# yamoling/lle

Measured on AMD Instinct MI355X. Metric: env-steps/s (agents x envs x steps/s), level-6 batch 65536, higher is better.
Workload: dtype u8

## Files before the change

lle_amd/csrc/obs_stream.hpp:

```cpp
#pragma once
#include <hip/hip_runtime.h>
#include <stdint.h>

#include <type_traits>

#include "tables.h"

namespace lle {

__device__ __forceinline__ void wave_sync() {
    __builtin_amdgcn_fence(__ATOMIC_RELEASE, "wavefront");
    __builtin_amdgcn_wave_barrier();
    __builtin_amdgcn_fence(__ATOMIC_ACQUIRE, "wavefront");
}

__device__ __forceinline__ uint32_t xcd_block(uint32_t b, uint32_t n_blocks) {
    const uint32_t x = b & 7u, q = n_blocks >> 3, r = n_blocks & 7u;
    return x * q + (x < r ? x : r) + (b >> 3);
}
__device__ __forceinline__ uint32_t xcd_block_dir(uint32_t b, uint32_t n_blocks, uint32_t flags) {
    const uint32_t blk = xcd_block(b, n_blocks);
    return (flags & LAUNCH_REVERSE) ? n_blocks - 1u - blk : blk;
}

__device__ __forceinline__ uint32_t row_rotation(uint32_t wave_id, uint32_t rows_per_wave, int64_t n_here, uint32_t flags) {
    const uint32_t r = wave_id & (rows_per_wave - 1u);
    return ((flags & LAUNCH_ROTATE_ROWS) && (int64_t)r < n_here && n_here == (int64_t)rows_per_wave) ? r : 0u;
}
__device__ __forceinline__ uint32_t rotated(uint32_t k, uint32_t rot, uint32_t n) {
    const uint32_t kk = k + rot;
    return kk >= n ? kk - n : kk;
}

typedef uint32_t u32x4 __attribute__((ext_vector_type(4)));
#define LLE_COPY_ROWS(SRC)                                                                                              \
    for (uint32_t r0 = wave_in_wg; r0 < rows; r0 += 8 * waves_per_wg) {                                                \
        const uint32_t r1 = r0 + waves_per_wg, r2 = r1 + waves_per_wg, r3 = r2 + waves_per_wg, r4 = r3 + waves_per_wg, \
                       r5 = r4 + waves_per_wg, r6 = r5 + waves_per_wg, r7 = r6 + waves_per_wg;                          \
        const u32x4 z = {0, 0, 0, 0};                                                                                   \
        u32x4 v0 = SRC(r0), v1 = z, v2 = z, v3 = z, v4 = z, v5 = z, v6 = z, v7 = z;                                      \
        if (r1 < rows) v1 = SRC(r1);                                                                                    \
        if (r2 < rows) v2 = SRC(r2);                                                                                    \
        if (r3 < rows) v3 = SRC(r3);                                                                                    \
        if (r4 < rows) {                                                                                                \
            v4 = SRC(r4);                                                                                               \
            if (r5 < rows) v5 = SRC(r5);                                                                                \
            if (r6 < rows) v6 = SRC(r6);                                                                                \
            if (r7 < rows) v7 = SRC(r7);                                                                                \
        }                                                                                                               \
        __builtin_amdgcn_sched_barrier(0);                        \
        dst[r0 * 64] = v0;                                                                                              \
        if (r1 < rows) dst[r1 * 64] = v1;                                                                               \
        if (r2 < rows) dst[r2 * 64] = v2;                                                                               \
        if (r3 < rows) dst[r3 * 64] = v3;                                                                               \
        if (r4 < rows) {                                                                                                \
            dst[r4 * 64] = v4;                                                                                          \
            if (r5 < rows) dst[r5 * 64] = v5;                                                                           \
            if (r6 < rows) dst[r6 * 64] = v6;                                                                           \
            if (r7 < rows) dst[r7 * 64] = v7;                                                                           \
        }                                                                                                               \
    }
__device__ __forceinline__ void copy_tables_to_lds(const uint8_t* __restrict__ tables, uint8_t* lds, uint32_t tab_bytes,
                                                   uint32_t lane, uint32_t wave_in_wg, uint32_t waves_per_wg) {
    const u32x4* __restrict__ src = reinterpret_cast<const u32x4*>(tables) + lane;
    u32x4* dst = reinterpret_cast<u32x4*>(lds) + lane;
    const uint32_t rows = tab_bytes / 1024;
#define LLE_SRC1(r) src[(r) * 64]
    LLE_COPY_ROWS(LLE_SRC1)
#undef LLE_SRC1
}

__device__ __forceinline__ void copy_tables2_to_lds(const uint8_t* __restrict__ t1, uint32_t bytes1, const uint8_t* __restrict__ t2, uint32_t bytes2,
                                                    uint8_t* lds, uint32_t lane, uint32_t wave_in_wg, uint32_t waves_per_wg) {
    const u32x4* __restrict__ s1 = reinterpret_cast<const u32x4*>(t1) + lane;
    const u32x4* __restrict__ s2 = reinterpret_cast<const u32x4*>(t2) + lane;
    u32x4* dst = reinterpret_cast<u32x4*>(lds) + lane;
    const uint32_t rows1 = bytes1 / 1024, rows = rows1 + bytes2 / 1024;
#define LLE_SRC2(r) (*((r) < rows1 ? s1 + (r) * 64 : s2 + ((r) - rows1) * 64))
    LLE_COPY_ROWS(LLE_SRC2)
#undef LLE_SRC2
}
#undef LLE_COPY_ROWS

__device__ __forceinline__ void expand_packed_tables(const uint8_t* __restrict__ pk, uint8_t* lds, uint32_t HW, uint32_t n_lay, uint32_t lds_meta, uint32_t lds_dyn,
                                                     uint32_t tail_bytes, uint32_t tid, uint32_t T) {
    const uint64_t* __restrict__ m4 = reinterpret_cast<const uint64_t*>(pk);
    const uint16_t* __restrict__ idx = reinterpret_cast<const uint16_t*>(pk + packed_meta_bytes(HW));
    const uint64_t* __restrict__ lay = reinterpret_cast<const uint64_t*>(pk + packed_meta_bytes(HW) + packed_idx_bytes(n_lay));
    const uint4* __restrict__ tail = reinterpret_cast<const uint4*>(pk + packed_meta_bytes(HW) + packed_idx_bytes(n_lay) + ((n_lay * 8u + 15u) & ~15u));
    const uint32_t n4 = (HW + 3u) / 4u, nt = tail_bytes / 16u;
    const uint64_t w0 = tid < n4 ? m4[tid] : 0ull;
    const uint32_t i0 = tid < n_lay ? (uint32_t)idx[tid] : 0u;
    const uint64_t l0 = tid < n_lay ? lay[tid] : 0ull;
    uint4 t0 = {0u, 0u, 0u, 0u};
    if (tid < nt) t0 = tail[tid];
    auto widen = [](uint64_t w) { return uint4{(uint32_t)w & 0xFFFFu, (uint32_t)(w >> 16) & 0xFFFFu, (uint32_t)(w >> 32) & 0xFFFFu, (uint32_t)(w >> 48)}; };
    uint4* z = reinterpret_cast<uint4*>(lds);
    for (uint32_t i = tid; i < lds_meta / 16u; i += T) z[i] = uint4{0u, 0u, 0u, 0u};
    uint4* md = reinterpret_cast<uint4*>(lds + lds_meta);
    if (tid < n4) md[tid] = widen(w0);
    for (uint32_t i = tid + T; i < n4; i += T) md[i] = widen(m4[i]);
    uint4* td = reinterpret_cast<uint4*>(lds + lds_dyn);
    if (tid < nt) td[tid] = t0;
    for (uint32_t i = tid + T; i < nt; i += T) td[i] = tail[i];
    asm volatile("s_waitcnt lgkmcnt(0)\n\ts_barrier" ::: "memory");
    uint64_t* ld = reinterpret_cast<uint64_t*>(lds);
    if (tid < n_lay) ld[i0] = l0;
    for (uint32_t i = tid + T; i < n_lay; i += T) ld[idx[i]] = lay[i];
}

__device__ __forceinline__ uint32_t mad24(uint32_t a, uint32_t b, uint32_t c) {
    uint32_t r;
    asm("v_mad_u32_u24 %0, %1, %2, %3" : "=v"(r) : "v"(a), "v"(b), "v"(c));
    return r;
}

template <typename T>
__device__ __forceinline__ void small_store(T* p, T v) {
#ifdef LLE_SMALL_WT
    if constexpr (sizeof(T) == 1) {
        asm volatile("global_store_byte %0, %1, off sc1" ::"v"(p), "v"((uint32_t)(uint8_t)v) : "memory");
    } else if constexpr (sizeof(T) == 2) {
        asm volatile("global_store_short %0, %1, off sc1" ::"v"(p), "v"((uint32_t)(uint16_t)v) : "memory");
    } else if constexpr (sizeof(T) == 4) {
        uint32_t w;
        __builtin_memcpy(&w, &v, 4);
        asm volatile("global_store_dword %0, %1, off sc1" ::"v"(p), "v"(w) : "memory");
    } else {
        static_assert(sizeof(T) == 8, "small_store: 1, 2, 4 or 8 bytes");
        uint64_t w;
        __builtin_memcpy(&w, &v, 8);
        asm volatile("global_store_dwordx2 %0, %1, off sc1" ::"v"(p), "v"(w) : "memory");
    }
#else
    *p = v;
#endif
}

template <bool WT>
__device__ __forceinline__ void stream_store(uint4* p, const uint4& v) {
    if constexpr (WT) {
        const u32x4 w = {v.x, v.y, v.z, v.w};
        asm volatile("global_store_dwordx4 %0, %1, off sc1\n\ts_nop 1" ::"v"(p), "v"(w));
    } else {
        *p = v;
    }
}

template <bool WT>
__device__ __forceinline__ void stream_row(uint4* __restrict__ dst, const uint4* srcv, uint32_t first, uint32_t n_chunks, uint32_t lane) {
    uint32_t c = first + lane;
    for (; c + 192u < n_chunks; c += 256u) {
        const uint4 q0 = srcv[c], q1 = srcv[c + 64u], q2 = srcv[c + 128u], q3 = srcv[c + 192u];
        stream_store<WT>(dst + c, q0);
        stream_store<WT>(dst + c + 64u, q1);
        stream_store<WT>(dst + c + 128u, q2);
        stream_store<WT>(dst + c + 192u, q3);
    }
    for (; c < n_chunks; c += 64u) stream_store<WT>(dst + c, srcv[c]);
}

template <bool WT>
__device__ __forceinline__ void stream_whole_row(uint4* __restrict__ dst, const uint4* srcv, uint32_t n_chunks, uint32_t lane) {
    const uint32_t c0 = lane, c1 = lane + 64u;
    const uint4 v0 = srcv[c0 < n_chunks ? c0 : 0u], v1 = srcv[c1 < n_chunks ? c1 : 0u];
    if (c0 < n_chunks) stream_store<WT>(dst + c0, v0);
    if (c1 < n_chunks) stream_store<WT>(dst + c1, v1);
    if (n_chunks > 128u) stream_row<WT>(dst, srcv, 128u, n_chunks, lane);
}

template <bool WT>
__device__ __forceinline__ void stream_row_tail(uint4* __restrict__ dst, const uint4* srcv, uint32_t n_chunks, uint32_t head_lo, uint32_t head_n,
                                                uint32_t lane, uint32_t head2_lo = 0, uint32_t head2_n = 0) {
    const uint32_t n_tail = n_chunks - head_n - head2_n;
    auto chunk_of = [&](uint32_t i) {
        uint32_t c = i + (i >= head_lo ? head_n : 0u);
        if (head2_n) c += c >= head2_lo ? head2_n : 0u;
        return c;
    };
    const uint32_t i0 = lane, i1 = lane + 64u;
    const uint32_t c0 = chunk_of(i0), c1 = chunk_of(i1);
    const uint4 v0 = srcv[i0 < n_tail ? c0 : 0u], v1 = srcv[i1 < n_tail ? c1 : 0u];
    if (i0 < n_tail) stream_store<WT>(dst + c0, v0);
    if (i1 < n_tail) stream_store<WT>(dst + c1, v1);
    for (uint32_t i = lane + 128u; i < n_tail; i += 64u) {
        const uint32_t c = chunk_of(i);
        stream_store<WT>(dst + c, srcv[c]);
    }
}

template <bool WT>
__device__ __forceinline__ void stream_row_dyn(uint4* __restrict__ dst, const uint4* srcv, const uint16_t* tab, uint32_t n_dyn, uint32_t c0, uint32_t c1,
                                               uint32_t lane) {
    const uint4 v0 = srcv[c0 != 0xFFFFu ? c0 : 0u], v1 = srcv[c1 != 0xFFFFu ? c1 : 0u];
    if (c0 != 0xFFFFu) stream_store<WT>(dst + c0, v0);
    if (c1 != 0xFFFFu) stream_store<WT>(dst + c1, v1);
    for (uint32_t i = lane + 128u; i < n_dyn; i += 64u) {
        const uint32_t c = tab[i];
        stream_store<WT>(dst + c, srcv[c]);
    }
}

__device__ __forceinline__ uint4 widen_chunk16(const int8_t* tmpl, uint32_t q, uint32_t one, uint32_t sel_lo, uint32_t sel_hi) {
    const uint2 w = reinterpret_cast<const uint2*>(tmpl)[q];
    uint32_t o[4];
#pragma unroll
    for (int k = 0; k < 4; k++) {
        const uint32_t src = k < 2 ? w.x : w.y;
        const uint32_t x = __builtin_amdgcn_perm(src, src, (k & 1) ? sel_hi : sel_lo);
        o[k] = __umul24(x & 0x00010001u, one) | ((x & 0x00800080u) << 8);
    }
    return make_uint4(o[0], o[1], o[2], o[3]);
}
__device__ __forceinline__ uint4 widen_chunk32(const int8_t* tmpl, uint32_t q) {
    const uint32_t w = reinterpret_cast<const uint32_t*>(tmpl)[q];
    uint32_t o[4];
#pragma unroll
    for (int k = 0; k < 4; k++) {
        const uint32_t b = (w >> (8 * k)) & 0xFFu;
        o[k] = ((b & 1u) ? 0x3F800000u : 0u) | ((b & 0x80u) << 24);
    }
    return make_uint4(o[0], o[1], o[2], o[3]);
}
struct WideConsts { uint32_t one, sel_lo, sel_hi, sh, lane; };
__device__ __forceinline__ WideConsts wide_consts(uint32_t et, uint32_t lane) {
    uint32_t z = 0;
    asm volatile("" : "+s"(z));
    asm volatile("" : "+v"(lane));
    WideConsts c;
    c.one = (et == OBS_F16 ? 0x3C00u : 0x3F80u) | z;
    c.sel_lo = 0x0c010c00u | z;
    c.sel_hi = 0x0c030c02u | z;
    c.sh = obs_elem_shift(et) + z;
    c.lane = lane;
    return c;
}
template <bool WT>
__device__ __forceinline__ void stream_wide(uint4* __restrict__ dst, const int8_t* tmpl, uint32_t n_chunks, uint32_t et, uint32_t lane_in) {
    const WideConsts c = wide_consts(et, lane_in);
    const uint32_t n_out = n_chunks << c.sh;
    if (c.sh == 2u) {
#pragma clang loop unroll(disable)
        for (uint32_t q = c.lane; q < n_out; q += 64u) stream_store<WT>(dst + q, widen_chunk32(tmpl, q));
    } else {
#pragma clang loop unroll(disable)
        for (uint32_t q = c.lane; q < n_out; q += 64u) stream_store<WT>(dst + q, widen_chunk16(tmpl, q, c.one, c.sel_lo, c.sel_hi));
    }
}
template <bool WT>
__device__ __forceinline__ void stream_wide_dyn(uint4* __restrict__ dst, const int8_t* tmpl, const uint16_t* tab, uint32_t t_lo, uint32_t t_hi, uint32_t c_base,
                                                uint32_t et, uint32_t lane_in) {
    const WideConsts c = wide_consts(et, lane_in);
#pragma clang loop unroll(disable)
    for (uint32_t i = (t_lo << c.sh) + c.lane; i < (t_hi << c.sh); i += 64u) {
        const uint32_t q = (((uint32_t)tab[i >> c.sh] - c_base) << c.sh) + (i & ((1u << c.sh) - 1u));
        stream_store<WT>(dst + q, c.sh == 2u ? widen_chunk32(tmpl, q) : widen_chunk16(tmpl, q, c.one, c.sel_lo, c.sel_hi));
    }
}

template <bool WT>
__device__ __forceinline__ void store_heads(int8_t* __restrict__ obs, uint64_t obs_stride, int64_t env0, int64_t n_here, uint32_t head_lo,
                                            uint32_t head_n, const uint4& v, uint32_t lane, uint32_t rot = 0, uint32_t head2_lo = 0, uint32_t head2_n = 0) {
    const uint32_t chunk = lane < head_n ? head_lo + lane : head2_lo + (lane - head_n);
    if (lane < head_n + head2_n)
        for (uint32_t k = 0; k < (uint32_t)n_here; k++)
            stream_store<WT>(reinterpret_cast<uint4*>(obs + (uint64_t)(env0 + rotated(k, rot, (uint32_t)n_here)) * obs_stride) + chunk, v);
}

template <bool CAN_WIDE, typename F>
__device__ __forceinline__ void dispatch_stream(uint32_t lflags, F&& f) {
    const bool wt = (lflags & LAUNCH_WRITE_THROUGH) != 0;
    if constexpr (CAN_WIDE) {
        if (lflags & LAUNCH_OBS_ELEM_MASK) {
            if (wt) f(std::true_type{}, std::true_type{});
            else f(std::false_type{}, std::true_type{});
            return;
        }
    }
    if (wt) f(std::true_type{}, std::false_type{});
    else f(std::false_type{}, std::false_type{});
}

template <bool WT, bool HEAD = false, bool INCR = false, bool WIDE = false>
__device__ __forceinline__ void write_observations(int A, int L, uint32_t D, uint32_t n_chunks, uint64_t obs_stride,
                                                   const uint64_t* dyn, int8_t* tmpl, const uint32_t* scratch,
                                                   uint32_t scr_stride, int8_t* __restrict__ obs, int64_t env0,
                                                   int64_t n_here, uint32_t lane, uint32_t head_lo = 0, uint32_t head_n = 0, uint32_t rot = 0,
                                                   const uint16_t* dyn_chunks = nullptr, uint32_t n_dyn_chunks = 0, uint32_t et = OBS_I8) {
    static_assert(!(WIDE && HEAD), "the kernels with row heads carry no widening code: the launcher never sends them a widened launch");
    uint32_t dc0 = 0xFFFFu, dc1 = 0xFFFFu;
    if constexpr (INCR) {
        dc0 = lane < n_dyn_chunks ? (uint32_t)dyn_chunks[lane] : 0xFFFFu;
        dc1 = lane + 64u < n_dyn_chunks ? (uint32_t)dyn_chunks[lane + 64u] : 0xFFFFu;
    }
    const bool has_d0 = lane < D;
    const uint64_t e0 = has_d0 ? dyn[lane] : 0ull;
    const uint32_t d0_idx = dyn_index(e0);
    const int32_t d0_base = dyn_base(e0);
    const uint32_t d0_refs = dyn_refs(e0), d0_gem = dyn_gem(e0);
    const uint32_t d0_r0 = dyn_ref0(e0), d0_r1 = dyn_ref1(e0);
    const uint32_t d0_w0 = d0_refs >= 1 ? 1u + ref_word(d0_r0) : 0u, d0_s0 = d0_refs >= 1 ? ref_bit(d0_r0) : 0u;
    const uint32_t d0_w1 = d0_refs >= 2 ? 1u + ref_word(d0_r1) : 0u, d0_s1 = d0_refs >= 2 ? ref_bit(d0_r1) : 0u;
    const uint32_t d0_wg = d0_gem != NO_GEM ? (uint32_t)L + 1u : 0u, d0_sg = d0_gem != NO_GEM ? gem_bit(d0_gem) : 0u;
    const bool is_agent_lane = (int)lane < A;
    const uint4* srcv = reinterpret_cast<const uint4*>(tmpl);

    for (uint32_t k0 = 0; k0 < (uint32_t)n_here; k0++) {
        const uint32_t k = rotated(k0, rot, (uint32_t)n_here);
        const uint32_t* sc = scratch + k * scr_stride;
        {
            const uint32_t lit = ((sc[d0_w0] >> d0_s0) | (sc[d0_w1] >> d0_s1) | (sc[d0_wg] >> d0_sg)) & 1u;
            if (has_d0) tmpl[d0_idx] = (int8_t)(lit ? 1 : d0_base);
        }
        for (uint32_t d = lane + 64u; d < D; d += 64) {
            const uint64_t e = dyn[d];
            const uint32_t refs = dyn_refs(e), gem = dyn_gem(e);
            const uint32_t r0 = dyn_ref0(e), r1 = dyn_ref1(e);
            const uint32_t w0 = refs >= 1 ? 1u + ref_word(r0) : 0u, w1 = refs >= 2 ? 1u + ref_word(r1) : 0u;
            const uint32_t wg = gem != NO_GEM ? (uint32_t)L + 1u : 0u;
            const uint32_t lit = ((sc[w0] >> (refs >= 1 ? ref_bit(r0) : 0u)) | (sc[w1] >> (refs >= 2 ? ref_bit(r1) : 0u)) |
                                  (sc[wg] >> (gem != NO_GEM ? gem_bit(gem) : 0u))) & 1u;
            tmpl[dyn_index(e)] = (int8_t)(lit ? 1 : dyn_base(e));
        }
        const uint32_t agent_idx = is_agent_lane ? sc[L + 2 + lane] : 0u;
        if (is_agent_lane) tmpl[agent_idx] = 1;
        wave_sync();
        uint4* __restrict__ dst = reinterpret_cast<uint4*>(obs + (uint64_t)(env0 + k) * obs_stride);
        if constexpr (WIDE) {
            if constexpr (INCR) stream_wide_dyn<WT>(dst, tmpl, dyn_chunks, 0u, n_dyn_chunks, 0u, et, lane);
            else stream_wide<WT>(dst, tmpl, n_chunks, et, lane);
        } else if constexpr (INCR) stream_row_dyn<WT>(dst, srcv, dyn_chunks, n_dyn_chunks, dc0, dc1, lane);
        else if constexpr (HEAD) stream_row_tail<WT>(dst, srcv, n_chunks, head_lo, head_n, lane);
        else stream_whole_row<WT>(dst, srcv, n_chunks, lane);
        wave_sync();
        if (is_agent_lane) tmpl[agent_idx] = 0;
    }
}

template <bool WT, bool INCR = false, bool WIDE = false>
__device__ __forceinline__ void write_observations_split(int A, int L, uint32_t D, uint32_t lo, uint32_t hi, uint64_t obs_stride,
                                                         const uint64_t* dyn, int8_t* tmpl, const uint32_t* records,
                                                         uint32_t scr_stride, int8_t* __restrict__ obs, int64_t wg_env0,
                                                         int64_t n_wg_here, uint32_t lane, const uint16_t* dyn_chunks = nullptr, uint32_t n_dyn_chunks = 0,
                                                         uint32_t et = OBS_I8) {
    const uint32_t b_lo = lo * 16u, b_hi = hi * 16u;
    uint32_t t_lo = 0, t_hi = 0;
    if constexpr (INCR) {
        for (uint32_t i = lane; i < ((n_dyn_chunks + 63u) & ~63u); i += 64) {
            const uint32_t c = i < n_dyn_chunks ? (uint32_t)dyn_chunks[i] : 0xFFFFFFFFu;
            t_lo += (uint32_t)__popcll(__ballot(c < lo));
            t_hi += (uint32_t)__popcll(__ballot(c < hi));
        }
    }
    uint32_t d_lo = 0, d_hi = 0;
    for (uint32_t d = lane; d < ((D + 63u) & ~63u); d += 64) {
        const uint32_t idx = d < D ? dyn_index(dyn[d]) : 0xFFFFFFFFu;
        d_lo += (uint32_t)__popcll(__ballot(idx < b_lo));
        d_hi += (uint32_t)__popcll(__ballot(idx < b_hi));
    }
    const bool has_d0 = d_lo + lane < d_hi;
    const uint64_t e0 = has_d0 ? dyn[d_lo + lane] : 0ull;
    const uint32_t d0_idx = has_d0 ? dyn_index(e0) - b_lo : 0u;
    const int32_t d0_base = dyn_base(e0);
    const uint32_t d0_refs = dyn_refs(e0), d0_gem = dyn_gem(e0);
    const uint32_t d0_r0 = dyn_ref0(e0), d0_r1 = dyn_ref1(e0);
    const uint32_t d0_w0 = d0_refs >= 1 ? 1u + ref_word(d0_r0) : 0u, d0_s0 = d0_refs >= 1 ? ref_bit(d0_r0) : 0u;
    const uint32_t d0_w1 = d0_refs >= 2 ? 1u + ref_word(d0_r1) : 0u, d0_s1 = d0_refs >= 2 ? ref_bit(d0_r1) : 0u;
    const uint32_t d0_wg = d0_gem != NO_GEM ? (uint32_t)L + 1u : 0u, d0_sg = d0_gem != NO_GEM ? gem_bit(d0_gem) : 0u;
    const bool is_agent_lane = (int)lane < A;
    const uint4* srcv = reinterpret_cast<const uint4*>(tmpl);
    const uint32_t n_mine = hi - lo;

    for (int64_t k = 0; k < n_wg_here; k++) {
        const uint32_t* sc = records + (uint32_t)k * scr_stride;
        {
            const uint32_t lit = ((sc[d0_w0] >> d0_s0) | (sc[d0_w1] >> d0_s1) | (sc[d0_wg] >> d0_sg)) & 1u;
            if (has_d0) tmpl[d0_idx] = (int8_t)(lit ? 1 : d0_base);
        }
        for (uint32_t d = d_lo + lane + 64u; d < d_hi; d += 64) {
            const uint64_t e = dyn[d];
            const uint32_t refs = dyn_refs(e), gem = dyn_gem(e);
            const uint32_t r0 = dyn_ref0(e), r1 = dyn_ref1(e);
            const uint32_t w0 = refs >= 1 ? 1u + ref_word(r0) : 0u, w1 = refs >= 2 ? 1u + ref_word(r1) : 0u;
            const uint32_t wg = gem != NO_GEM ? (uint32_t)L + 1u : 0u;
            const uint32_t lit = ((sc[w0] >> (refs >= 1 ? ref_bit(r0) : 0u)) | (sc[w1] >> (refs >= 2 ? ref_bit(r1) : 0u)) |
                                  (sc[wg] >> (gem != NO_GEM ? gem_bit(gem) : 0u))) & 1u;
            tmpl[dyn_index(e) - b_lo] = (int8_t)(lit ? 1 : dyn_base(e));
        }
        const uint32_t agent_idx = is_agent_lane ? sc[L + 2 + lane] : 0xFFFFFFFFu;
        const bool agent_here = agent_idx >= b_lo && agent_idx < b_hi;
        if (agent_here) tmpl[agent_idx - b_lo] = 1;
        wave_sync();
        uint4* __restrict__ dst = reinterpret_cast<uint4*>(obs + (uint64_t)(wg_env0 + k) * obs_stride) + ((uint64_t)lo << (WIDE ? obs_elem_shift(et) : 0u));
        if constexpr (WIDE) {
            if constexpr (INCR) stream_wide_dyn<WT>(dst, tmpl, dyn_chunks, t_lo, t_hi, lo, et, lane);
            else stream_wide<WT>(dst, tmpl, n_mine, et, lane);
        } else if constexpr (INCR) {
            for (uint32_t i = t_lo + lane; i < t_hi; i += 64u) {
                const uint32_t c = (uint32_t)dyn_chunks[i] - lo;
                stream_store<WT>(dst + c, srcv[c]);
            }
        } else {
            stream_whole_row<WT>(dst, srcv, n_mine, lane);
        }
        wave_sync();
        if (agent_here) tmpl[agent_idx - b_lo] = 0;
    }
}

__device__ __forceinline__ void elem_eval(uint32_t e, const uint32_t* sc, int A, int L, uint32_t HW, const uint8_t* laser_layer,
                                          uint32_t gem_layer, uint32_t& idx, int32_t& val, bool& on) {
    const uint32_t cell = elem_cell(e), i5 = elem_index(e), off = elem_bit(e), type = elem_type(e);
    const uint32_t colour = (sc[L + 2 + A + (i5 >> 2)] >> ((i5 & 3u) * 8u)) & 0xFFu;
    const bool is_gem = type == ELEM_GEM;
    const uint32_t llayer = laser_layer ? (uint32_t)laser_layer[colour] : (uint32_t)A + colour;
    idx = (is_gem ? gem_layer : llayer) * HW + cell;
    val = type == ELEM_SOURCE ? -1 : 1;
    on = type == ELEM_SOURCE ? true : (is_gem ? ((sc[L + 1] >> i5) & 1u) != 0 : ((sc[1 + i5] >> off) & 1u) != 0);
}
template <bool WT, bool HEAD = false, bool INCR = false, bool WIDE = false>
__device__ __forceinline__ void write_observations_env(int A, int L, uint32_t HW, uint32_t n_elems, uint32_t n_chunks,
// ... 66 lines not shown
```

lle_amd/csrc/step_kernel.hpp:

```cpp
#pragma once
#include "kernel_common.hpp"
#include "partial_stream.hpp"
#include "step_lanes.hpp"

namespace lle {


__device__ __forceinline__ EnvOutputs load_uniform(const EnvOutputs* p) {
    static_assert(sizeof(EnvOutputs) == 64, "one s_load_dwordx16");
    typedef uint32_t u32x16 __attribute__((ext_vector_type(16)));
    u32x16 w;
    asm volatile("s_load_dwordx16 %0, %1, 0x0\n\ts_waitcnt lgkmcnt(0)" : "=s"(w) : "s"(p) : "memory");
    EnvOutputs o;
    __builtin_memcpy(&o, &w, sizeof o);
    return o;
}

constexpr size_t KERNARG_ENV_OUT = ((sizeof(BatchPtrs) + alignof(LaunchArgs) - 1) / alignof(LaunchArgs)) * alignof(LaunchArgs) + offsetof(LaunchArgs, out);
__device__ __forceinline__ const EnvOutputs* kernarg_env_out() {
    return reinterpret_cast<const EnvOutputs*>((const char*)__builtin_amdgcn_kernarg_segment_ptr() + KERNARG_ENV_OUT);
}

template <int G, int LM, int MODE, bool ML1, int LX = -1>
__global__ void __launch_bounds__(256, (G >= 8 ? 3 : 4)) step_kernel(BatchPtrs P, LaunchArgs K) {
    constexpr bool PARTIAL = MODE == 9;
    constexpr bool GEN = (MODE >= 2 && MODE <= 5) || MODE == 7 || MODE == 8 || PARTIAL, ROLL = MODE >= 1 && MODE <= 3;
    constexpr bool PES = MODE == 3 || MODE == 5 || MODE == 8;
    constexpr bool BM = LM >= 8;
    constexpr int LR = BM ? 1 : LM;
    constexpr bool CAN_SPLIT = G >= 8 && !PES && !PARTIAL;
    constexpr bool HEAD = MODE == 6 || MODE == 7 || MODE == 8;
    const bool split = CAN_SPLIT && (K.flags & LAUNCH_SPLIT_ROWS) != 0;
#ifdef LLE_STAMP_SINGLE
    constexpr bool STAMPED = true;
#else
    constexpr bool STAMPED = ROLL;
#endif
    uint64_t* const stamps = STAMPED ? K.stamps : nullptr;
#undef LLE_STAMP
#define LLE_STAMP(i)                                                                              \
    do {                                                                                          \
        if (STAMPED && stamps && lane == 0) stamps[(uint64_t)wave_id * 8 + (i)] = __builtin_amdgcn_s_memrealtime(); \
    } while (0)
    const uint32_t EPW = K.envs_per_wave < (uint32_t)(64 / G) ? K.envs_per_wave : (uint32_t)(64 / G);
    constexpr int NW = (2 * G + 7) / 8;
    extern __shared__ __attribute__((aligned(16))) uint8_t lds[];
    const uint32_t lane = threadIdx.x & 63u, wave_in_wg = threadIdx.x >> 6, waves_per_wg = blockDim.x >> 6;
    const uint32_t blk = xcd_block_dir(blockIdx.x, gridDim.x, K.flags);
    const uint32_t wave_id = blk * waves_per_wg + wave_in_wg;
    const uint8_t* __restrict__ tables = P.tables;
    const InitRecord* __restrict__ initp = P.init;
    uint32_t map_idx = 0u;
    if (GEN) {
        const uint32_t EPW0 = K.envs_per_wave < (uint32_t)(64 / G) ? K.envs_per_wave : (uint32_t)(64 / G);
        map_idx = map_index_of(K, K.env_base + (int64_t)(blk * waves_per_wg) * EPW0);
        tables += (uint64_t)map_idx * K.table_stride;
        initp += map_idx;
    }
    const MapHeader* __restrict__ hdr = reinterpret_cast<const MapHeader*>(tables);
    const int A = (int)hdr->A, L = LX >= 0 ? LX : (int)hdr->L, W = (int)hdr->W;
    const uint32_t a = lane & (G - 1), grp = lane / G;
    const int64_t As = agent_stride_of(A, L);
    const int64_t env0 = K.env_base + (int64_t)wave_id * EPW;
    const int64_t env = env0 + grp;
    const bool env_ok = grp < EPW && env < K.env_limit;
    const bool me = env_ok && (int)a < A;
    const bool write_obs = !PARTIAL && hdr->obs_supported && !(K.flags & STEP_NO_OBS);
    const uint32_t h_HW = hdr->HW, h_obs_stride = hdr->obs_stride, h_n_chunks = hdr->n_chunks, h_D = hdr->D;
#define LLE_ET() (HEAD ? (uint32_t)OBS_I8 : (K.flags & LAUNCH_OBS_ELEM_MASK) >> LAUNCH_OBS_ELEM_SHIFT)
#define LLE_PITCH() ((uint64_t)h_obs_stride << obs_elem_shift(LLE_ET()))
    uint32_t h_beam_full[LR];
#pragma unroll
    for (int b = 0; b < LR; b++) h_beam_full[b] = (!BM && b < L) ? hdr->beam_full[b] : 0u;
    const uint32_t h_enabled = hdr->enabled_mask;
    const uint32_t h_chain = BM ? hdr->chain_mask : 0u;
    const uint32_t h_off_cell_meta = hdr->off_cell_meta, h_off_dyn = hdr->off_dyn, h_off_template = hdr->off_template;
    const uint32_t h_max_layers = ML1 ? 1u : hdr->max_layers;
    constexpr bool CAN_INCR = !ROLL && !PARTIAL && !HEAD;
    const uint32_t h_off_dyn_chunks = CAN_INCR ? (PES ? hdr->off_pes_dyn_chunks : hdr->off_dyn_chunks) : 0u;
    const uint32_t h_n_dyn_chunks = CAN_INCR ? (PES ? hdr->n_pes_dyn_chunks : hdr->n_dyn_chunks) : 0u;
    const bool incr = CAN_INCR && (K.flags & STEP_INCREMENTAL_OBS) != 0 && h_n_dyn_chunks < h_n_chunks;
    const uint32_t h_off_recolour = PES ? hdr->off_recolour : 0u, h_off_bare = PES ? hdr->off_bare : 0u;
    const uint32_t h_off_elems = PES ? hdr->off_elems : 0u, h_n_elems = PES ? hdr->n_elems : 0u;
    constexpr bool ENV_OUT = MODE == 4 || MODE == 5 || MODE == 7 || MODE == 8 || PARTIAL;
    EnvOutputs O_early = {};
    uint32_t h_G = 0, h_H = 0;
    constexpr bool EARLY_OUT = MODE == 7;
    if (EARLY_OUT && K.env_out) O_early = K.out;
    if (ENV_OUT) { h_G = hdr->G; h_H = hdr->H; }
    uint32_t h_init_beams[LR];
#pragma unroll
    for (int b = 0; b < LR; b++) h_init_beams[b] = (!BM && b < L) ? initp->beams[b] : 0u;
    const int64_t n_here = (K.env_limit - env0) < (int64_t)EPW ? (K.env_limit - env0) : (int64_t)EPW;
    const uint32_t amask = (1u << A) - 1u;
#define LLE_ROT() ((ROLL && PES) ? 0u : row_rotation(wave_id, EPW, n_here, K.flags))
    LLE_STAMP(0);

    uint32_t pos = 0xFFFF0000u + a, avail = 0, beams[LR];
    uint64_t raw_bits = 0;
    uint32_t gems = 0;
#pragma unroll
    for (int b = 0; b < LR; b++) beams[b] = 0;
    const int64_t env_c = env_ok ? env : 0;
    uint64_t* const p_bits = P.bits + env_c;
    uint32_t* const p_gems = P.gems + env_c;
    uint32_t* const p_beams = P.beams + env_c * L;
    uint16_t* const p_pos = P.pos + env_c * As + a;
    uint8_t* const p_avail = P.avail + env_c * As + a;
    uint8_t* const p_err = P.err + env_c;
    uint8_t* const p_evcount = P.evcount + env_c;
    uint8_t* const p_events = P.events + env_c * 2 * As;
    uint8_t* const p_done = P.done + env_c;
#define LLE_LATE(field, offset) ((GEN || ROLL) ? P.field + (offset) : p_##field)
#define LLE_ENV_LATE(name)                                   \
    int64_t name = env_c;                                    \
    if ((GEN || ROLL) && !HEAD) asm volatile("" : "+v"(name))
    uint32_t init_pos_a = 0xFFFF0000u + a, init_avail_a = 0;
    uint64_t init_bits = 0;
    uint32_t init_gems = 0;
    constexpr int CWM = LM / 4;
    const int CW = src_stride_of(L) / 4;
    uint32_t colw[CWM], env_enabled = h_enabled;
    constexpr bool PRE_BEAMS = PES && !ROLL && LM <= 8;
    const bool shared_init = PES && !ROLL && hdr->recolour_exact != 0u;
    uint32_t env_init_beams[LR];
#pragma unroll
    for (int b = 0; b < LR; b++) env_init_beams[b] = 0u;
#pragma unroll
    for (int q = 0; q < CWM; q++) colw[q] = 0;
    uint32_t act_given = 4u;
    constexpr int BPL = (HEAD && BM) ? (LM + G - 1) / G : 1;
    uint32_t bm_pre[BPL];
#pragma unroll
    for (int k = 0; k < BPL; k++) bm_pre[k] = 0u;
    constexpr bool PRE_STATS = (MODE == 0 || MODE == 6 || MODE == 7 || MODE == 8) && LM <= 8;
    int64_t stats_old = 0;
#define LLE_LOAD_STATE() \
    do { \
        if (env_ok) { \
            raw_bits = *p_bits; \
            gems = *p_gems; \
        _Pragma("unroll") \
            for (int b = 0; b < LR; b++) \
                if (!BM && b < L) beams[b] = p_beams[b]; \
        } \
        if (me) { \
            pos = (uint32_t)*p_pos; \
            avail = (uint32_t)*p_avail; \
            init_pos_a = (PES && !shared_init) ? (uint32_t)P.init_pos[env * As + a] : (uint32_t)initp->pos[a]; \
            init_avail_a = (PES && !shared_init) ? (uint32_t)P.init_avail[env * As + a] : (uint32_t)initp->avail[a]; \
            if (!ROLL && !(K.flags & STEP_SAMPLE_ACTIONS)) \
                act_given = K.actions_in ? (uint32_t)K.actions_in[env * A + a] : (uint32_t)P.actions[env * As + a]; \
        } \
        if (HEAD && BM && env_ok) { \
        _Pragma("unroll") \
            for (int k = 0; k < BPL; k++) \
                if ((int)a + k * G < L) bm_pre[k] = p_beams[(int)a + k * G]; \
        } \
        init_bits = initp->bits; \
        init_gems = initp->gems; \
        if (PRE_STATS) stats_old = stats_preload(P.stats, wave_id, lane); \
        if (PES && env_ok) { \
            env_enabled = P.src_enabled[env]; \
        _Pragma("unroll") \
            for (int q = 0; q < CWM; q++) \
                if (q < CW) colw[q] = reinterpret_cast<const uint32_t*>(P.src_colour)[env * CW + q]; \
            if ((K.flags & STEP_AUTO_RESET) && !shared_init) { \
                init_bits = P.init_bits[env]; \
                init_gems = P.init_gems[env]; \
        _Pragma("unroll") \
                for (int b = 0; b < LR; b++) \
                    if (PRE_BEAMS && b < L) env_init_beams[b] = P.init_beams[env * L + b]; \
            } \
        } \
    } while (0)

    const uint32_t head_lo = HEAD ? (PES ? hdr->pes_head_lo : hdr->head_lo) : 0u;
    const uint32_t head_n = (HEAD && write_obs && !split && !incr) ? (PES ? hdr->pes_head_n : hdr->head_n) : 0u;
    const uint32_t head2_lo = (HEAD && PES) ? hdr->pes_head2_lo : 0u, head2_n = (HEAD && PES && head_n) ? hdr->pes_head2_n : 0u;
    uint4 head_v = {0u, 0u, 0u, 0u};
    if (HEAD) {
        if (lane < head_n + head2_n)
            head_v = reinterpret_cast<const uint4*>(tables + (PES ? h_off_bare : h_off_template))[lane < head_n ? head_lo + lane : head2_lo + (lane - head_n)];
        LLE_LOAD_STATE();
    }
    uint32_t bt_full = 0u, bt_init = 0u;
    if (BM && (int)threadIdx.x < L) {
        bt_full = hdr->beam_full[threadIdx.x];
        bt_init = initp->beams[threadIdx.x];
    }
    const uint32_t tab_off = hdr->off_cell_lay;
    const uint32_t tab_cells = ((hdr->off_dyn - tab_off) + 1023u) & ~1023u;
    const uint32_t tab_bytes = PARTIAL ? (tab_cells < hdr->lds_table_bytes ? tab_cells : hdr->lds_table_bytes)
                                       : (split ? hdr->lds_split_table_bytes : hdr->lds_table_bytes);
    const bool use_sets = PARTIAL && K.win_sets != nullptr;
    const uint32_t ext_bytes = PES ? hdr->ext_bytes : (use_sets ? win_sets_bytes(hdr->HW) : 0u);
    constexpr int PB = CAN_SPLIT ? 8 : 1;
    const uint32_t cpw = (h_n_chunks + waves_per_wg - 1u) / waves_per_wg;
    const uint32_t c_lo = wave_in_wg * cpw < h_n_chunks ? wave_in_wg * cpw : h_n_chunks;
    const uint32_t c_hi = c_lo + cpw < h_n_chunks ? c_lo + cpw : h_n_chunks;
    uint32_t pre_bits[PB];
    uint32_t pre_neg = 0xFFFFFFFFu;
#pragma unroll
    for (int q = 0; q < PB; q++) pre_bits[q] = 0u;
    if (CAN_SPLIT && split) {
        const uint16_t* __restrict__ bits = reinterpret_cast<const uint16_t*>(tables + sizeof(MapHeader)) + c_lo;
#pragma unroll
        for (int q = 0; q < PB; q++)
            if (lane + 64u * q < c_hi - c_lo) pre_bits[q] = bits[lane + 64u * q];
        if (lane < TMPL_NEG_MAX) pre_neg = reinterpret_cast<const uint32_t*>(tables + sizeof(MapHeader) + tmpl_bits_bytes(h_n_chunks))[lane];
        if (!HEAD) LLE_LOAD_STATE();
    }
    if (PES) copy_tables2_to_lds(tables + tab_off, tab_bytes, tables + h_off_bare, ext_bytes, lds, lane, wave_in_wg, waves_per_wg);
    else if (use_sets) copy_tables2_to_lds(tables + tab_off, tab_bytes, K.win_sets + (uint64_t)map_idx * win_table_bytes(hdr->HW), ext_bytes, lds, lane, wave_in_wg, waves_per_wg);
    else if (CAN_SPLIT && GEN && split && (K.flags & LAUNCH_PACKED_TABLES))
        expand_packed_tables(tables + hdr->off_packed, lds, h_HW, hdr->packed_n_lay, h_off_cell_meta - tab_off, h_off_dyn - tab_off, h_off_template - h_off_dyn,
                             threadIdx.x, blockDim.x);
    else copy_tables_to_lds(tables + tab_off, lds, tab_bytes, lane, wave_in_wg, waves_per_wg);
    constexpr uint32_t bt_bytes = BM ? 2u * LM * 4u : 0u;
    uint32_t* beam_tab = reinterpret_cast<uint32_t*>(lds + tab_bytes + ext_bytes);
    if (BM && (int)threadIdx.x < L) {
        beam_tab[threadIdx.x] = bt_full;
        beam_tab[LM + threadIdx.x] = bt_init;
    }
    const uint32_t pm_bytes = PARTIAL ? (use_sets ? 0u : partial_bitmap_bytes(hdr->H, (uint32_t)W)) + 32u : 0u;
    uint32_t* const part_bm = reinterpret_cast<uint32_t*>(lds + tab_bytes + ext_bytes + bt_bytes);
    uint8_t* const part_col = lds + tab_bytes + ext_bytes + bt_bytes + (pm_bytes - 32u);
    if (PARTIAL) {
        for (uint32_t w = threadIdx.x; w < (pm_bytes - 32u) / 4u; w += blockDim.x) part_bm[w] = 0u;
        if ((int)threadIdx.x < L) part_col[threadIdx.x] = hdr->beam_colour[threadIdx.x];
    }
    LLE_STAMP(7);
    if (HEAD) {
        __builtin_amdgcn_s_waitcnt(0x0F70);
        const uint32_t hgroup = MODE != 6 ? 1u : ((K.flags & LAUNCH_HEAD_GROUP4) ? 4u : ((K.flags & LAUNCH_HEAD_GROUP2) ? 2u : 1u));
        if (hgroup == 1u) {
            if (head_n && n_here > 0) {
                if (K.flags & LAUNCH_WRITE_THROUGH) store_heads<true>(P.obs, h_obs_stride, env0, n_here, head_lo, head_n, head_v, lane, LLE_ROT(), head2_lo, head2_n);
                else store_heads<false>(P.obs, h_obs_stride, env0, n_here, head_lo, head_n, head_v, lane, LLE_ROT(), head2_lo, head2_n);
            }
            asm volatile("s_waitcnt lgkmcnt(0)\n\ts_barrier" ::: "memory");
        } else {
            asm volatile("s_waitcnt lgkmcnt(0)\n\ts_barrier" ::: "memory");
            if (head_n && (wave_in_wg & (hgroup - 1u)) == 0u) {
                for (uint32_t q = 0; q < hgroup && wave_in_wg + q < waves_per_wg; q++) {
                    const int64_t e0q = env0 + (int64_t)q * EPW;
                    int64_t nq = K.env_limit - e0q;
                    nq = nq < 0 ? 0 : (nq > (int64_t)EPW ? (int64_t)EPW : nq);
                    if (nq > 0) {
                        if (K.flags & LAUNCH_WRITE_THROUGH) store_heads<true>(P.obs, h_obs_stride, e0q, nq, head_lo, head_n, head_v, lane);
                        else store_heads<false>(P.obs, h_obs_stride, e0q, nq, head_lo, head_n, head_v, lane);
                    }
                }
            }
        }
    } else {
        __syncthreads();
        if (!(CAN_SPLIT && split)) LLE_LOAD_STATE();
    }

    const uint64_t* cell_lay = reinterpret_cast<const uint64_t*>(lds);
    const uint32_t* cell_meta = reinterpret_cast<const uint32_t*>(lds + (h_off_cell_meta - tab_off));
    const uint64_t* dyn = reinterpret_cast<const uint64_t*>(lds + (h_off_dyn - tab_off));
    const uint16_t* dyn_chunks = PES ? reinterpret_cast<const uint16_t*>(lds + tab_bytes + (h_off_dyn_chunks - h_off_bare))
                                     : reinterpret_cast<const uint16_t*>(lds + (h_off_dyn_chunks - tab_off));
    const uint32_t scr_stride = (uint32_t)(L + A + 2 + (PES ? CW : 0)) | 1u;
    const uint32_t part_pitch = PARTIAL ? (((uint32_t)(A * (2 * A + 3)) * K.partial_k * K.partial_k + 15u) & ~15u) : 0u;
    const uint32_t row_area = PARTIAL ? K.partial_E * part_pitch + 16u : h_obs_stride;
    const uint32_t priv_bytes = row_area + (PARTIAL ? ((EPW * scr_stride * 4u + 15u) & ~15u) : 64u * scr_stride * 4u) + (PES ? PES_WAVE_EXTRA_BYTES : 0u);
    int8_t* tmpl = reinterpret_cast<int8_t*>(lds + tab_bytes + ext_bytes + bt_bytes + pm_bytes + wave_in_wg * priv_bytes);
    uint32_t* scratch = reinterpret_cast<uint32_t*>(tmpl + row_area);
    const int8_t* bare = reinterpret_cast<const int8_t*>(lds + tab_bytes);
    const uint32_t* elems = reinterpret_cast<const uint32_t*>(lds + tab_bytes + (h_off_elems - h_off_bare));
    if (split) {
        tmpl = reinterpret_cast<int8_t*>(lds + tab_bytes + bt_bytes + wave_in_wg * cpw * 16u);
        scratch = reinterpret_cast<uint32_t*>(lds + tab_bytes + bt_bytes + waves_per_wg * cpw * 16u) + wave_in_wg * EPW * scr_stride;
        uint4* mine = reinterpret_cast<uint4*>(tmpl);
        if (hdr->off_tmpl_bits) {
            auto expand = [](uint32_t b) {
                return uint4{((b & 15u) * 0x00204081u) & 0x01010101u, (((b >> 4) & 15u) * 0x00204081u) & 0x01010101u,
                             (((b >> 8) & 15u) * 0x00204081u) & 0x01010101u, ((b >> 12) * 0x00204081u) & 0x01010101u};
            };
#pragma unroll
            for (int q = 0; q < PB; q++)
                if (lane + 64u * q < c_hi - c_lo) mine[lane + 64u * q] = expand(pre_bits[q]);
            const uint16_t* __restrict__ bits = reinterpret_cast<const uint16_t*>(tables + sizeof(MapHeader)) + c_lo;
            for (uint32_t c = lane + 64u * PB; c < c_hi - c_lo; c += 64) mine[c] = expand(bits[c]);
            if (lane < hdr->tmpl_neg_n && pre_neg >= c_lo * 16u && pre_neg < c_hi * 16u) tmpl[pre_neg - c_lo * 16u] = (int8_t)-1;
        } else {
            const uint4* __restrict__ pristine = reinterpret_cast<const uint4*>(tables + h_off_template) + c_lo;
            for (uint32_t c = lane; c < c_hi - c_lo; c += 64) mine[c] = pristine[c];
        }
    } else if (PARTIAL) {
        if (!use_sets) partial_bitmap_fill(part_bm, cell_lay, cell_meta, (int)hdr->H, W);
    } else {
        const uint4* pristine = PES ? reinterpret_cast<const uint4*>(bare) : reinterpret_cast<const uint4*>(lds + (h_off_template - tab_off));
        uint4* mine = reinterpret_cast<uint4*>(tmpl);
        for (uint32_t c = lane; c < h_n_chunks; c += 64) mine[c] = pristine[c];
    }
    uint32_t* const bm = scratch + grp * scr_stride + 1;
    if (HEAD && BM) {
        if (env_ok) {
#pragma unroll
            for (int k = 0; k < BPL; k++)
                if ((int)a + k * G < L) bm[(int)a + k * G] = bm_pre[k];
        }
    } else if (BM && env_ok) {
        for (int b = (int)a; b < L; b += G) bm[b] = p_beams[b];
    }
    wave_sync();
    if (!HEAD) __builtin_amdgcn_s_waitcnt(0x0F70);
    LLE_STAMP(1);

    uint32_t alive = (uint32_t)raw_bits & 0xFFFFu, arrived = (uint32_t)(raw_bits >> 16) & 0xFFFFu, occ = (uint32_t)(raw_bits >> 32) & 0xFFFFu;
    uint32_t ghost = (uint32_t)(raw_bits >> GHOST_SHIFT);
    const uint32_t enabled = PES ? env_enabled : h_enabled, max_layers = h_max_layers;
    LLE_STAMP(2);

    StepCounts cnt = {0, 0, 0, 0, 0, 0, 0};
    constexpr bool CNT_LDS = ROLL && PES && G >= 2;
    uint32_t* const cnt_lds = scratch + 64u * scr_stride + grp * 8u;
    if (CNT_LDS && env_ok && a == 0) {
#pragma unroll
        for (int q = 0; q < 7; q++) cnt_lds[q] = 0u;
    }
    const uint32_t n_steps = ROLL ? (K.n_steps ? K.n_steps : 1u) : 1u;
    for (uint32_t it = 0; it < n_steps; it++) {
    const uint64_t t_now = K.t + it;
    uint8_t* __restrict__ actions_out = P.actions;
    uint32_t* __restrict__ reward_out = P.reward;
    int8_t* __restrict__ obs_out = P.obs;
    if (ROLL && K.ring_slots) {
        uint32_t slot = (uint32_t)K.ring_pos + it;
        while (slot >= K.ring_slots) slot -= K.ring_slots;
        actions_out = K.ring_actions + (int64_t)slot * K.ring_env_count * As;
        reward_out = K.ring_reward + (int64_t)slot * K.ring_env_count;
        obs_out = K.ring_obs + (int64_t)slot * K.ring_env_count * (int64_t)LLE_PITCH();
    }

    uint32_t was_reset = 0;
    if (K.flags & STEP_AUTO_RESET) {
        const bool over = env_ok && ((alive | ghost) != amask || arrived == amask);
        pos = (over && me) ? init_pos_a : pos;
        avail = (over && me) ? init_avail_a : avail;
        alive = over ? ((uint32_t)init_bits & 0xFFFFu) : alive;
        arrived = over ? ((uint32_t)(init_bits >> 16) & 0xFFFFu) : arrived;
        occ = over ? ((uint32_t)(init_bits >> 32) & 0xFFFFu) : occ;
        ghost = over ? 0u : ghost;
        gems = over ? init_gems : gems;
#pragma unroll
        for (int b = 0; b < LR; b++)
            if (!BM && b < L && !(PES && shared_init))
                beams[b] = over ? (PES ? (PRE_BEAMS ? env_init_beams[b] : P.init_beams[env_ok ? env * L + b : 0]) : h_init_beams[b]) : beams[b];
        if (BM && over && !(PES && shared_init))
            for (int b = (int)a; b < L; b += G) bm[b] = PES ? P.init_beams[env * L + b] : beam_tab[LM + b];
        if (PES && shared_init && __ballot(over) != 0ull) {
            const uint32_t* rtab0 = reinterpret_cast<const uint32_t*>(lds + tab_bytes + (h_off_recolour - h_off_bare));
            if (!BM) {
#pragma unroll
                for (int b = 0; b < LR; b++)
                    if (b < L) {
                        const uint32_t c = (colw[b >> 2] >> ((b & 3) * 8)) & 0xFFu;
                        const uint32_t m = ((env_enabled >> b) & 1u) ? rtab0[b * (A + 1) + 1 + (int)(c < (uint32_t)A ? c : 0u)] : 0u;
                        beams[b] = over ? m : beams[b];
                    }
            } else if (over) {
                for (int b = (int)a; b < L; b += G) {
                    const uint32_t c = (colw[b >> 2] >> ((b & 3) * 8)) & 0xFFu;
                    bm[b] = ((env_enabled >> b) & 1u) ? rtab0[b * (A + 1) + 1 + (int)(c < (uint32_t)A ? c : 0u)] : 0u;
                }
            }
        }
        was_reset = over ? 1u : 0u;
        if (PES && !ROLL && (K.flags & STEP_RECOLOUR_RESETS) && __ballot(over) != 0ull) {
            const uint32_t* rtab = reinterpret_cast<const uint32_t*>(lds + tab_bytes + (h_off_recolour - h_off_bare));
            const uint64_t rkey = action_step_key(K.seed ^ RECOLOUR_SALT, t_now);
#pragma unroll
            for (int b = 0; b < LM; b++) {
                if (b < L) {
                    const uint32_t* row = rtab + b * (A + 1);
                    const uint32_t ok = row[0] & amask;
                    const uint32_t field = action_field(action_hash_pair(rkey, (uint64_t)(K.env_offset + env), (uint32_t)b >> 1), (uint32_t)b);
                    const uint32_t k = (field * (uint32_t)__popc(ok)) >> 16;
                    const bool mine = ((ok >> a) & 1u) != 0u && (uint32_t)__popc(ok & ((1u << a) - 1u)) == k;
                    const uint32_t pick = grp_or<G>(mine ? a + 1u : 0u);
                    const uint32_t sh = (uint32_t)(b & 3) * 8u, old_c = (colw[b >> 2] >> sh) & 0xFFu;
                    const uint32_t c = (over && pick) ? pick - 1u : old_c;
                    colw[b >> 2] = (colw[b >> 2] & ~(0xFFu << sh)) | (c << sh);
                    if (over && a == 0) P.init_beams[env * L + b] = ((env_enabled >> b) & 1u) ? row[1u + (c < (uint32_t)A ? c : 0u)] : 0u;
                }
// ... 307 lines not shown
```

Before: 13.19 billion.

## Issue head stores and state loads early in MODE 6 prologue via buffer ops

For MODE 6 (head-template mode), the kernel now issues all per-env state loads, the table-row loads (as raw buffer loads) and the observation head stores together in one prologue before waiting, instead of copying tables to LDS, waiting and then storing. The goal is to overlap global memory latency of state loads, LDS table fills and head stores. It also disables the split-rows path for this mode and adds a wrap-aware buffer store for rotated rows, which adds register pressure and code complexity.

```diff
diff --git a/lle_amd/csrc/obs_stream.hpp b/lle_amd/csrc/obs_stream.hpp
--- a/lle_amd/csrc/obs_stream.hpp
+++ b/lle_amd/csrc/obs_stream.hpp
@@ -82,6 +82,32 @@
 }
 #undef LLE_COPY_ROWS
 
+constexpr int BUFFER_RSRC_FLAGS = 0x00020000;
+template <int N>
+struct TableRows { u32x4 v[N]; };
+template <int N>
+__device__ __forceinline__ TableRows<N> request_table_rows(const uint8_t* tables, uint32_t tab_bytes, uint32_t lane, uint32_t wave_in_wg, uint32_t waves_per_wg) {
+    const __amdgpu_buffer_rsrc_t rsrc = __builtin_amdgcn_make_buffer_rsrc(const_cast<uint8_t*>(tables), 0, (int)tab_bytes, BUFFER_RSRC_FLAGS);
+    const uint32_t off = wave_in_wg * 1024u + lane * 16u, step = waves_per_wg * 1024u;
+    TableRows<N> t;
+#pragma unroll
+    for (int k = 0; k < N; k++) t.v[k] = __builtin_amdgcn_raw_buffer_load_b128(rsrc, (int)(off + (uint32_t)k * step), 0, 0);
+    return t;
+}
+template <int N>
+__device__ __forceinline__ void write_table_rows(const TableRows<N>& t, const uint8_t* __restrict__ tables, uint8_t* lds, uint32_t tab_bytes, uint32_t lane,
+                                                 uint32_t wave_in_wg, uint32_t waves_per_wg) {
+    u32x4* dst = reinterpret_cast<u32x4*>(lds) + lane;
+    const uint32_t rows = tab_bytes / 1024;
+#pragma unroll
+    for (int k = 0; k < N; k++) {
+        const uint32_t r = wave_in_wg + (uint32_t)k * waves_per_wg;
+        if (r < rows) dst[r * 64] = t.v[k];
+    }
+    const u32x4* __restrict__ src = reinterpret_cast<const u32x4*>(tables) + lane;
+    for (uint32_t r = wave_in_wg + (uint32_t)N * waves_per_wg; r < rows; r += waves_per_wg) dst[r * 64] = src[r * 64];
+}
+
 __device__ __forceinline__ void expand_packed_tables(const uint8_t* __restrict__ pk, uint8_t* lds, uint32_t HW, uint32_t n_lay, uint32_t lds_meta, uint32_t lds_dyn,
                                                      uint32_t tail_bytes, uint32_t tid, uint32_t T) {
     const uint64_t* __restrict__ m4 = reinterpret_cast<const uint64_t*>(pk);
@@ -267,6 +293,23 @@
             stream_store<WT>(reinterpret_cast<uint4*>(obs + (uint64_t)(env0 + rotated(k, rot, (uint32_t)n_here)) * obs_stride) + chunk, v);
 }
 
+template <bool WT, int ROWS>
+__device__ __forceinline__ void store_heads_early(int8_t* row0, uint32_t pitch, uint32_t n_here, uint32_t head_lo, uint32_t head_n, const u32x4& v,
+                                                  uint32_t lane, uint32_t rot) {
+    const uint32_t size = n_here * pitch;
+    const __amdgpu_buffer_rsrc_t rsrc = __builtin_amdgcn_make_buffer_rsrc(row0, 0, (int)size, BUFFER_RSRC_FLAGS);
+    const uint32_t wrap = rot ? size : 0xFFFFFFFFu;
+    uint32_t t = (lane < head_n ? (head_lo + lane) * 16u : 0x80000000u) + rot * pitch;
+    asm volatile("" : "+v"(t));
+#pragma unroll
+    for (int k = 0; k < ROWS; k++) {
+        const uint32_t w = t - wrap;
+        __builtin_amdgcn_raw_buffer_store_b128(v, rsrc, (int)(t < w ? t : w), 0, WT ? 16 : 0);
+        t += pitch;
+        __builtin_amdgcn_sched_barrier(0);
+    }
+}
+
 template <bool CAN_WIDE, typename F>
 __device__ __forceinline__ void dispatch_stream(uint32_t lflags, F&& f) {
     const bool wt = (lflags & LAUNCH_WRITE_THROUGH) != 0;
diff --git a/lle_amd/csrc/step_kernel.hpp b/lle_amd/csrc/step_kernel.hpp
--- a/lle_amd/csrc/step_kernel.hpp
+++ b/lle_amd/csrc/step_kernel.hpp
@@ -30,7 +30,8 @@
     constexpr int LR = BM ? 1 : LM;
     constexpr bool CAN_SPLIT = G >= 8 && !PES && !PARTIAL;
     constexpr bool HEAD = MODE == 6 || MODE == 7 || MODE == 8;
-    const bool split = CAN_SPLIT && (K.flags & LAUNCH_SPLIT_ROWS) != 0;
+    constexpr bool EARLY = MODE == 6;
+    const bool split = CAN_SPLIT && !EARLY && (K.flags & LAUNCH_SPLIT_ROWS) != 0;
 #ifdef LLE_STAMP_SINGLE
     constexpr bool STAMPED = true;
 #else
@@ -178,14 +179,15 @@
     const uint32_t head_lo = HEAD ? (PES ? hdr->pes_head_lo : hdr->head_lo) : 0u;
     const uint32_t head_n = (HEAD && write_obs && !split && !incr) ? (PES ? hdr->pes_head_n : hdr->head_n) : 0u;
     const uint32_t head2_lo = (HEAD && PES) ? hdr->pes_head2_lo : 0u, head2_n = (HEAD && PES && head_n) ? hdr->pes_head2_n : 0u;
+    const uint32_t hgroup = MODE != 6 ? 1u : ((K.flags & LAUNCH_HEAD_GROUP4) ? 4u : ((K.flags & LAUNCH_HEAD_GROUP2) ? 2u : 1u));
     uint4 head_v = {0u, 0u, 0u, 0u};
-    if (HEAD) {
+    if (HEAD && !EARLY) {
         if (lane < head_n + head2_n)
             head_v = reinterpret_cast<const uint4*>(tables + (PES ? h_off_bare : h_off_template))[lane < head_n ? head_lo + lane : head2_lo + (lane - head_n)];
         LLE_LOAD_STATE();
     }
     uint32_t bt_full = 0u, bt_init = 0u;
-    if (BM && (int)threadIdx.x < L) {
+    if (BM && !EARLY && (int)threadIdx.x < L) {
         bt_full = hdr->beam_full[threadIdx.x];
         bt_init = initp->beams[threadIdx.x];
     }
@@ -211,7 +213,77 @@
         if (lane < TMPL_NEG_MAX) pre_neg = reinterpret_cast<const uint32_t*>(tables + sizeof(MapHeader) + tmpl_bits_bytes(h_n_chunks))[lane];
         if (!HEAD) LLE_LOAD_STATE();
     }
-    if (PES) copy_tables2_to_lds(tables + tab_off, tab_bytes, tables + h_off_bare, ext_bytes, lds, lane, wave_in_wg, waves_per_wg);
+    if (EARLY) {
+        const uint32_t wave_u = blk * waves_per_wg + __builtin_amdgcn_readfirstlane(wave_in_wg);
+        const int64_t env0_u = K.env_base + (int64_t)wave_u * EPW;
+        int64_t nh = K.env_limit - env0_u;
+        nh = nh < 0 ? 0 : (nh > (int64_t)EPW ? (int64_t)EPW : nh);
+        const uint32_t rot_u = EPW == (uint32_t)(64 / G) ? row_rotation(wave_u, EPW, nh, K.flags) : 0u;
+        int8_t* const row0 = P.obs + env0_u * (int64_t)h_obs_stride;
+        constexpr int TR = (G <= 4 && LM == 4) ? 4 : 8;
+        constexpr int NS = 64 / G < 63 ? 64 / G : 63;
+        auto prologue = [&](auto policy_) {
+            constexpr int POLICY = decltype(policy_)::value;
+            asm volatile("; prologue %0" ::"n"(POLICY) : "memory");
+            const u32x4 hv = reinterpret_cast<const u32x4*>(tables + h_off_template)[head_lo + (lane < head_n ? lane : 0u)];
+            const uint32_t a_c = (int)a < A ? a : 0u;
+            uint64_t l_bits = *p_bits;
+            uint32_t l_gems = *p_gems;
+            uint32_t l_beams[LR];
+#pragma unroll
+            for (int b = 0; b < LR; b++)
+                l_beams[b] = (BM || (LX >= 0 && b >= LX)) ? 0u : *(b < L ? p_beams + b : p_gems);
+            uint32_t l_pos = (uint32_t)P.pos[env_c * As + a_c], l_avail = (uint32_t)P.avail[env_c * As + a_c];
+            uint32_t l_ipos = (uint32_t)initp->pos[a_c], l_iavail = (uint32_t)initp->avail[a_c];
+            const uint8_t* const act_p = K.actions_in ? K.actions_in + (env_c * A + a_c) : P.actions + (env_c * As + a_c);
+            uint32_t l_act = (uint32_t)*act_p;
+            uint32_t l_bm[BPL];
+#pragma unroll
+            for (int k = 0; k < BPL; k++) l_bm[k] = (HEAD && BM) ? p_beams[(int)a + k * G < L ? (int)a + k * G : 0] : 0u;
+            int64_t l_stats = PRE_STATS ? P.stats[(int64_t)wave_id * 8 + (lane & 7u)] : 0;
+            const uint32_t t_c = (int)threadIdx.x < L ? threadIdx.x : 0u;
+            uint32_t l_btf = BM ? hdr->beam_full[t_c] : 0u, l_bti = BM ? initp->beams[t_c] : 0u;
+            uint64_t l_ib = initp->bits;
+            uint32_t l_ig = initp->gems;
+            const TableRows<TR> trows = request_table_rows<TR>(tables + tab_off, tab_bytes, lane, wave_in_wg, waves_per_wg);
+            __builtin_amdgcn_sched_barrier(0);
+            if constexpr (POLICY == 0) {
+                __builtin_amdgcn_s_waitcnt(0x0F70);
+                head_v = uint4{hv.x, hv.y, hv.z, hv.w};
+                asm volatile("" : "+v"(head_v.x), "+v"(head_v.y), "+v"(head_v.z), "+v"(head_v.w));
+            } else {
+                store_heads_early<POLICY == 2, 64 / G>(row0, h_obs_stride, (uint32_t)nh, head_lo, head_n, hv, lane, rot_u);
+                __builtin_amdgcn_sched_barrier(0);
+                __builtin_amdgcn_s_waitcnt(0x0F70 | (NS & 15) | ((NS >> 4) << 14));
+            }
+            asm volatile("" : "+v"(l_bits), "+v"(l_gems), "+v"(l_pos), "+v"(l_avail), "+v"(l_ipos), "+v"(l_iavail), "+v"(l_act), "+v"(l_stats), "+v"(l_ib), "+v"(l_ig),
+                         "+v"(l_btf), "+v"(l_bti));
+#pragma unroll
+            for (int b = 0; b < LR; b++) asm volatile("" : "+v"(l_beams[b]));
+#pragma unroll
+            for (int k = 0; k < BPL; k++) asm volatile("" : "+v"(l_bm[k]));
+            raw_bits = env_ok ? l_bits : 0ull;
+            gems = env_ok ? l_gems : 0u;
+#pragma unroll
+            for (int b = 0; b < LR; b++) beams[b] = (!BM && b < L && env_ok) ? l_beams[b] : 0u;
+            pos = me ? l_pos : pos;
+            avail = me ? l_avail : 0u;
+            init_pos_a = me ? l_ipos : init_pos_a;
+            init_avail_a = me ? l_iavail : 0u;
+            act_given = (me && !(K.flags & STEP_SAMPLE_ACTIONS)) ? l_act : 4u;
+#pragma unroll
+            for (int k = 0; k < BPL; k++) bm_pre[k] = (HEAD && BM && env_ok && (int)a + k * G < L) ? l_bm[k] : 0u;
+            stats_old = (PRE_STATS && lane < 8u) ? l_stats : 0;
+            init_bits = l_ib;
+            init_gems = l_ig;
+            bt_full = l_btf;
+            bt_init = l_bti;
+            write_table_rows<TR>(trows, tables + tab_off, lds, tab_bytes, lane, wave_in_wg, waves_per_wg);
+        };
+        if (hgroup != 1u) prologue(std::integral_constant<int, 0>{});
+        else if (K.flags & LAUNCH_WRITE_THROUGH) prologue(std::integral_constant<int, 2>{});
+        else prologue(std::integral_constant<int, 1>{});
+    } else if (PES) copy_tables2_to_lds(tables + tab_off, tab_bytes, tables + h_off_bare, ext_bytes, lds, lane, wave_in_wg, waves_per_wg);
     else if (use_sets) copy_tables2_to_lds(tables + tab_off, tab_bytes, K.win_sets + (uint64_t)map_idx * win_table_bytes(hdr->HW), ext_bytes, lds, lane, wave_in_wg, waves_per_wg);
     else if (CAN_SPLIT && GEN && split && (K.flags & LAUNCH_PACKED_TABLES))
         expand_packed_tables(tables + hdr->off_packed, lds, h_HW, hdr->packed_n_lay, h_off_cell_meta - tab_off, h_off_dyn - tab_off, h_off_template - h_off_dyn,
@@ -232,10 +304,9 @@
     }
     LLE_STAMP(7);
     if (HEAD) {
-        __builtin_amdgcn_s_waitcnt(0x0F70);
-        const uint32_t hgroup = MODE != 6 ? 1u : ((K.flags & LAUNCH_HEAD_GROUP4) ? 4u : ((K.flags & LAUNCH_HEAD_GROUP2) ? 2u : 1u));
+        if (!EARLY) __builtin_amdgcn_s_waitcnt(0x0F70);
         if (hgroup == 1u) {
-            if (head_n && n_here > 0) {
+            if (!EARLY && head_n && n_here > 0) {
                 if (K.flags & LAUNCH_WRITE_THROUGH) store_heads<true>(P.obs, h_obs_stride, env0, n_here, head_lo, head_n, head_v, lane, LLE_ROT(), head2_lo, head2_n);
                 else store_heads<false>(P.obs, h_obs_stride, env0, n_here, head_lo, head_n, head_v, lane, LLE_ROT(), head2_lo, head2_n);
             }
```

Result: no change. 13.32 billion, median of 6 (+1.0%).
